# BGI-Qingdao/HAST

Measured on AMD Instinct MI355X. Metric: classified read-bp/sec at k=21, 150bp reads, 200M unique-mers/hap, higher is better.
Workload: dtype u64; 1 GPU; C3 human-trio scale: 200M+200M synthetic 21-mers, 10M barcodes, 150bp reads; k=21, read_len=150, keys_per_hap=200000000, barcodes=10000000, batch_reads=48000000, reads_total=5760000000, minimizer=16, keys=random, collective=none (D2H of counters in timed region), resident_batches=12

## Files before the change

### hast_amd/binding.py

```python
import ctypes as C
import os
import subprocess

import numpy as np

_HERE = os.path.dirname(os.path.abspath(__file__))
_LIB = None

u8p, u32p, u64p, vp = C.POINTER(C.c_uint8), C.POINTER(C.c_uint32), C.POINTER(C.c_uint64), C.c_void_p

STATUS = {0: "OK", 1: "INVALID", 2: "NO_DEVICE", 3: "HIP", 4: "OOM", 5: "TABLE_FULL", 6: "FORMAT", 7: "RCCL", 8: "IO", 9: "UNSUPPORTED"}


class SynthParams(C.Structure):
    _fields_ = [("seed_k", C.c_uint64), ("seed_r", C.c_uint64), ("seed_b", C.c_uint64),
                ("n_keys_per_hap", C.c_uint64), ("n_barcodes", C.c_uint32), ("read_len", C.c_uint32),
                ("k", C.c_uint32), ("reserved", C.c_uint32)]


class KcSynth(C.Structure):
    _fields_ = [("seed", C.c_uint64), ("genome_len", C.c_uint64), ("read_len", C.c_uint32), ("snp_per_1024", C.c_uint32),
                ("err_per_4096", C.c_uint32), ("n_per_4096", C.c_uint32)]


# ... 72 lines not shown
    "hast_dev_free": (C.c_int, [vp, vp]),
    "hast_memcpy_h2d": (C.c_int, [vp, vp, vp, C.c_size_t]),
    "hast_memcpy_d2h": (C.c_int, [vp, vp, vp, C.c_size_t]),
    "hast_memset_d": (C.c_int, [vp, vp, C.c_int, C.c_size_t, vp]),
    "hast_table_reserve": (C.c_int, [vp, C.c_uint64, C.c_double]),
    "hast_table_insert_text": (C.c_int, [vp, C.c_int, C.c_char_p, C.c_size_t, u64p]),
    "hast_table_insert_text_file": (C.c_int, [vp, C.c_int, C.c_char_p, u64p]),
    "hast_ctx_set_text_check": (C.c_int, [vp, C.c_int]),
    "hast_table_insert_keys": (C.c_int, [vp, C.c_int, vp, C.c_size_t]),
    "hast_table_insert_keys_device": (C.c_int, [vp, C.c_int, vp, C.c_size_t, vp]),
    "hast_table_erase": (C.c_int, [vp, vp, C.c_size_t, vp]),
    "hast_table_sizes": (C.c_int, [vp, u64p, u64p]),
    "hast_table_lookup": (C.c_int, [vp, vp, C.c_size_t, vp]),
    "hast_table_save": (C.c_int, [vp, C.c_char_p]),
    "hast_table_load": (C.c_int, [vp, C.c_char_p, C.c_double]),
    "hast_table_file_info": (C.c_int, [C.c_char_p, C.POINTER(C.c_int), u64p]),
    "hast_table_info": (C.c_int, [vp, u64p, u64p]),
    "hast_table_clone": (C.c_int, [vp, vp]),
    "hast_ctx_set_filter": (C.c_int, [vp, C.c_int, C.c_int, C.c_int, C.c_int]),
    "hast_filter_build": (C.c_int, [vp]),
    "hast_filter_info": (C.c_int, [vp, C.POINTER(C.c_int), C.POINTER(C.c_int), C.POINTER(C.c_int), C.POINTER(C.c_int), u64p]),
    "hast_filter_dense": (C.c_int, [vp, C.POINTER(C.c_int)]),
    "hast_filter_request_ceiling": (C.c_int, [vp, C.POINTER(C.c_double)]),
    "hast_counts_resize": (C.c_int, [vp, C.c_size_t]),
    "hast_counts_bind": (C.c_int, [vp, vp, C.c_size_t]),
    "hast_counts_zero": (C.c_int, [vp, vp]),
    "hast_counts_read": (C.c_int, [vp, vp, vp, vp, C.c_size_t]),
    "hast_counts_pack": (C.c_int, [vp, vp, C.c_size_t, vp]),
    "hast_counts_unpack": (C.c_int, [vp, vp, C.c_size_t, vp]),
    "hast_counts_add_votes": (C.c_int, [vp, vp, vp, C.c_size_t, C.c_uint32, vp]),
    "hast_counts_allreduce": (C.c_int, [C.POINTER(vp), C.c_int]),
    "hast_classify_timing": (C.c_int, [vp, C.c_int]),
    "hast_classify_times": (C.c_int, [vp, C.POINTER(C.c_float), C.POINTER(C.c_float), C.c_int, C.POINTER(C.c_int)]),
    "hast_classify_device": (C.c_int, [vp, vp, C.c_size_t, vp, C.c_uint32, vp, vp, C.c_size_t, vp]),
    "hast_classify_batch": (C.c_int, [vp, vp, vp, vp, C.c_size_t, C.c_uint32]),
    "hast_classify_perread_device": (C.c_int, [vp, vp, C.c_size_t, vp, C.c_size_t, vp, vp]),
    "hast_classify_perread": (C.c_int, [vp, vp, vp, C.c_size_t, vp]),
    "hast_batch_begin": (C.c_int, [vp, C.c_size_t, C.c_size_t, C.POINTER(vp), C.POINTER(vp), C.POINTER(vp)]),
    "hast_batch_submit": (C.c_int, [vp, C.c_size_t, C.c_uint32]),
    "hast_names_create": (C.c_int, [vp, C.c_size_t, C.POINTER(vp)]),
    "hast_names_destroy": (None, [vp]),
    "hast_fq_create": (C.c_int, [vp, C.c_size_t, C.c_int, vp, C.POINTER(vp)]),
    "hast_fq_create_ex": (C.c_int, [vp, C.c_size_t, C.c_int, vp, C.c_int, C.POINTER(vp)]),
    "hast_fq_create_striped": (C.c_int, [C.POINTER(vp), C.c_int, C.c_size_t, C.c_int, C.POINTER(vp), C.POINTER(vp)]),
    "hast_fq_create_striped_ex": (C.c_int, [C.POINTER(vp), C.c_int, C.c_size_t, C.c_int, C.POINTER(vp), C.c_int, C.POINTER(vp)]),
    "hast_fq_lanes": (C.c_int, [vp]),
# ... 245 lines not shown
    def filter_build(self):
        _ck(self._lib.hast_filter_build(self._h))

    def filter_request_ceiling(self):
        r = C.c_double()
        _ck(self._lib.hast_filter_request_ceiling(self._h, C.byref(r)))
        return r.value

    def filter_info(self):
        en, m, t, kp, b = C.c_int(), C.c_int(), C.c_int(), C.c_int(), C.c_uint64()
        _ck(self._lib.hast_filter_info(self._h, C.byref(en), C.byref(m), C.byref(t), C.byref(kp), C.byref(b)))
        return bool(en.value), m.value, t.value, kp.value, b.value

    def filter_mode(self):
        en = C.c_int()
        _ck(self._lib.hast_filter_info(self._h, C.byref(en), None, None, None, None))
        return en.value

    def filter_dense(self):
        d = C.c_int()
        _ck(self._lib.hast_filter_dense(self._h, C.byref(d)))
        return bool(d.value)

    def close(self):
        if self._h:
            self._lib.hast_ctx_destroy(self._h)
            self._h = C.c_void_p()

    def __enter__(self):
        return self

    def __exit__(self, *a):
        self.close()

    def __del__(self):
        try:
            self.close()
        except Exception:
            pass

    @property
    def stream(self):
        return self._lib.hast_ctx_stream(self._h)

    def sync(self, stream=None):
        _ck(self._lib.hast_stream_sync(self._h, stream))
# ... 551 lines not shown
```

### hast_amd/csrc/classify_main.cpp

```cpp
#include <getopt.h>
#include <sys/stat.h>
#include <unistd.h>

#include <algorithm>
#include <atomic>
#include <cerrno>
#include <chrono>
#include <deque>
#include <cstdarg>
#include <cstdio>
#include <cstdlib>
#include <cstring>
#include <ctime>
#include <condition_variable>
#include <memory>
#include <mutex>
#include <string>
#include <thread>
#include <string_view>
#include <unordered_map>
#include <vector>

#include "../../include/hast.h"
#include "fq_feed.h"
// ... 1773 lines not shown
    if (o.stats && rs.naming.device_dict)
        stat_line("__stats_dictionary__ on=device dictionaries=%zu ids_limit=%zu ids_from_device=%zu ids_from_host=%zu merge_by_text_s=%.3f texts_merged_to_host=%zu rows_summed_by_text=%zu\n", rs.naming.groups.size(), rs.naming.host_base, rs.n_dev_names, rs.n_host_names, rs.naming.merge_s,
                  rs.naming.merged_to_host, rs.n_rows_summed);
    if (o.stats) {
        const char *nc = getenv("HAST_NAME_CACHE"), *rb = getenv("HAST_GZ_RING_BYTES"), *pg = getenv("HAST_PARK_GB");
        stat_line("__stats_sizes__ name_cache=%s gz_ring_bytes=%s park_gb=%s\n", nc ? nc : "default", rb ? rb : "default", pg ? pg : "default");
    }
    if (o.stats) stat_line("__stats_setup__ waited_for_stream_setup_s=%.3f (inside scrub_sizes_clone_s: .gz inputs opened, FASTQ streams created while the table was built)\n", rs.t_pre_waited);
    for (size_t i = 0; i < rs.ctxs.size(); i++) {
        char sw[512] = "";
        (void)hast_ctx_options(rs.ctxs[i], sw, sizeof(sw));
        if (strstr(sw, "filter_fallback"))
            fprintf(stderr, " WARN : GPU %d (context %zu) had no room for the k-mer filter and probed the table directly (%s)\n", o.devices[i], i, sw);
    }
    if (o.stats) {
        char sw[512] = "";
        (void)hast_ctx_options(rs.ctx, sw, sizeof(sw));
        stat_line("__stats_switches__ %s\n", sw[0] ? sw : "none");
        int f_on = 0, f_m = 0, f_t = 0, f_kp = 0;
        uint64_t f_bytes = 0;
        (void)hast_filter_info(rs.ctx, &f_on, &f_m, &f_t, &f_kp, &f_bytes);
        stat_line("__stats_filter__ mode=%s m=%d t=%d kp=%d bytes=%llu\n", f_on == 2 ? "exact_entries" : f_on == 1 ? "prints" : "off_table_only", f_m, f_t, f_kp,
                  (unsigned long long)f_bytes);
    }
    if (rs.hbm_thread.joinable()) {
        rs.hbm_stop = true;
        rs.hbm_thread.join();
        size_t parked = 0;
        (void)hast_dev_mem_info(rs.ctx, nullptr, nullptr, &parked);
        const size_t fm = rs.hbm_free_min.load(), tot = rs.hbm_total.load();
        if (tot) stat_line("__stats_hbm__ total_bytes=%zu free_min_bytes=%zu in_use_peak_bytes=%zu parked_bytes_at_end=%zu\n", tot, fm, tot - std::min(fm, tot), parked);
    }
    fprintf(stderr, "__END__\n");
    rs.t_printed = now_s();
}

int leave(Run &rs) {
    const Options &o = rs.o;
    const char *preload = getenv("LD_PRELOAD");
    const bool profiled = getenv("ROCP_TOOL_LIBRARIES") || (preload && strstr(preload, "rocprofiler"));
    if (!getenv("HAST_TEARDOWN") && !profiled) {
        if (o.stats) stat_phases(rs, nullptr);
        if (!o.stats_json.empty() && !write_stats_json(o.stats_json)) fprintf(stderr, "classify: cannot write %s\n", o.stats_json.c_str());
        if (fflush(stdout) != 0) die_output();
        fflush(stderr);
        _exit(0);
// ... 51 lines not shown
```

### hast_amd/csrc/hast_api.cpp

```cpp
#include <dlfcn.h>
#include <fcntl.h>
#include <sys/stat.h>
#include <unistd.h>
#include <hip/hip_runtime.h>

#include <algorithm>
#include <chrono>
#include <atomic>
#include <cstdarg>
#include <cstdio>
#include <cstdlib>
#include <cstring>
#include <functional>
#include <map>
#include <mutex>
#include <new>
#include <string>
#include <vector>

#include "../../include/hast.h"
#include "hast_common.h"
#include "hast_device.h"
#include "kc_device.h"
#include "fq_device.h"
// ... 13 lines not shown
    size_t cap_bases = 0, cap_reads = 0;
    hipEvent_t done = nullptr;
    bool in_flight = false;
};

}

struct hast_ctx {
    int device = 0;
    int k = 0;
    int m = 0;
    int n_cu = 256;
    hipStream_t stream = nullptr;
    uint64_t *d_slots = nullptr;
    uint32_t nbuckets = 0;
    unsigned long long *d_counts = nullptr;
    uint32_t *h_errword = nullptr;
    unsigned long long *d_pack = nullptr;
    size_t pack_words = 0;
    size_t n_barcodes = 0;
    bool counts_owned = false;
    uint32_t *d_err = nullptr;
    unsigned long long *d_cnt = nullptr;
    void *d_scratch = nullptr;
    size_t scratch_bytes = 0;
    Staging stage[2];
    unsigned batch_no = 0;
    void *d_seg = nullptr;
    size_t seg_bytes = 0;
    std::vector<hipEvent_t> t_ev;
    size_t t_slots = 0, t_next = 0, t_count = 0;
    uint32_t *d_votes_scratch = nullptr;
    size_t votes_bytes = 0;
    CommitScratch part;
    char *sf_h[2] = {nullptr, nullptr}, *sf_d[2] = {nullptr, nullptr};
    hipEvent_t sf_done[2] = {nullptr, nullptr};
    void *d_filter = nullptr;
    size_t filter_bytes = 0;
    FilterGeom fg{};
    bool filter_valid = false;
    bool use_filter = true;
    size_t filter_fallback_bytes = 0;
    bool test_filter_oom = false;
    int filter_m = 0, filter_t = 0, filter_kp = 0;
    int filter_exact = -1;
    int text_acgt_only = 0;
// ... 197 lines not shown
    if (device < 0 || device >= n) return set_error(HAST_ERR_NO_DEVICE, "device %d not in [0,%d)", device, n);
    HAST_HIP_TRY(hipSetDevice(device));
    tr("hipSetDevice");
    hast_ctx *c = new (std::nothrow) hast_ctx();
    if (!c) return set_error(HAST_ERR_OOM, "host allocation failed");
    c->device = device;
    c->k = k;
    c->m = default_minimizer(k);
    if (const char *e = getenv("HAST_CLASSIFY")) c->use_filter = strcmp(e, "exact") != 0;
    if (const char *e = getenv("HAST_TEST_FILTER_OOM")) c->test_filter_oom = atoi(e) != 0;
    if (const char *e = getenv("HAST_FILTER_M")) c->filter_m = atoi(e);
    if (const char *e = getenv("HAST_FILTER_T")) c->filter_t = atoi(e);
    if (const char *e = getenv("HAST_FILTER_KP")) c->filter_kp = atoi(e);
    if (const char *e = getenv("HAST_FILTER_EXACT")) {
        if (!strcmp(e, "once")) c->exact_env_once = true;
        else c->exact_env_off = atoi(e) == 0;
    }
    if (c->exact_env_off) c->filter_exact = 0;
    else if (c->exact_env_once) c->filter_exact = 1;
    if (const char *e = getenv("HAST_COMMIT")) c->commit_mode = !strcmp(e, "atomic") ? 1 : !strcmp(e, "partition") ? 2 : 0;
    if (const char *e = getenv("HAST_PART_SPAN")) c->part_span = (uint32_t)atoi(e);
    if (const char *e = getenv("HAST_F_GEO")) c->kernel_geo = e[0] != '0';
    if (const char *e = getenv("HAST_F_RL")) c->kernel_rl = e[0] != '0';
    if (const char *e = getenv("HAST_TILE_LDS")) {
        const long v = atol(e);
        if (v >= 4096 && v <= 160 * 1024) c->tile_lds = (size_t)v;
    }
    hipDeviceProp_t prop;
    if (hipGetDeviceProperties(&prop, device) == hipSuccess) c->n_cu = prop.multiProcessorCount;
    tr("hipGetDeviceProperties");
    hast_status st = HAST_OK;
    auto bail = [&](hipError_t he, const char *what) {
        if (he != hipSuccess && st == HAST_OK) st = set_error(HAST_ERR_HIP, "%s: %s", what, hipGetErrorString(he));
    };
    bail(hipStreamCreateWithFlags(&c->stream, hipStreamNonBlocking), "hipStreamCreate");
    tr("hipStreamCreate");
    bail(dev_malloc(&c->d_err, 4 * sizeof(uint32_t)), "dev_malloc(err)");
    tr("first hipMalloc");
    bail(dev_malloc(&c->d_cnt, 8 * sizeof(unsigned long long)), "dev_malloc(cnt)");
    bail(pinned_malloc(reinterpret_cast<void **>(&c->h_errword), 64, hipHostMallocDefault), "pinned_malloc(err word)");
    if (st == HAST_OK) bail(hipMemsetAsync(c->d_err, 0, 4 * sizeof(uint32_t), c->stream), "hipMemset");
    if (st == HAST_OK) bail(hipStreamSynchronize(c->stream), "hipStreamSynchronize");
    tr("first fill + synchronize");
    for (auto &s : c->stage)
        if (st == HAST_OK) bail(hipEventCreateWithFlags(&s.done, hipEventDisableTiming), "hipEventCreate");
    tr("events");
    if (st != HAST_OK) {
        hast_ctx_destroy(c);
        return st;
    }
    *out = c;
    return HAST_OK;
}

void hast_release_parked(void) { release_parked(); }

void hast_ctx_destroy(hast_ctx *c) {
    if (!c) return;
    (void)hipSetDevice(c->device);
    if (c->stream) (void)hipStreamSynchronize(c->stream);
    release_parked();
    for (auto &s : c->stage) {
        if (s.h_bases) (void)hipHostFree(s.h_bases);
        if (s.h_off) (void)hipHostFree(s.h_off);
// ... 787 lines not shown
    uint32_t tr = tr_max;
    if (a.max_pos > 0) {
        double best = -1;
        for (uint32_t t = tr_max; t >= 1 && t + 8 > tr_max; --t) {
            const uint64_t q = (uint64_t)t * a.max_pos, blocks = (q + 63) / 64, slots = filt ? (blocks + 3) / 4 * 4 : (blocks + 7) / 8 * 8;
            const double eff = (double)q / (double)(slots * 64);
            if (eff > best + 1e-9) { best = eff; tr = t; }
        }
    }
    a.tile_reads = tr;
    const size_t smem = per_read * tr + pad;
    if (smem + (filt ? (size_t)kTmerLevelTableWords * 4 : 0) > (160u << 10)) return set_error(HAST_ERR_INVALID, "read_len %u needs %zu B of LDS", read_len, smem);
    auto magic = [](uint64_t qmax, uint32_t d) -> uint32_t {
        if (d <= 1 || qmax * d >= (1ull << 32)) return 0;
        return (uint32_t)((1ull << 32) / d) + 1;
    };
    a.div_magic = magic((uint64_t)tr * a.max_pos + 1024, a.max_pos);
    a.div_mh = magic((uint64_t)tr * a.mh_stride + 1024, a.mh_stride);
    a.div_hw = magic((uint64_t)tr * a.w64 * 2 + 1024, a.w64 * 2);
    a.div_l1g = magic((uint64_t)tr * (a.l1_stride / 4) + 1024, a.l1_stride / 4);
    const uint64_t n_tiles = (n_reads + tr - 1) / tr;
    const int grid = (int)std::min<uint64_t>(n_tiles, (uint64_t)c->n_cu * 8);
    a.tile_queue = c->d_cnt + 3;
    HAST_HIP_TRY(hipMemsetAsync(a.tile_queue, 0, sizeof(unsigned long long), hs));
    hipEvent_t *ev = c->t_slots ? &c->t_ev[3 * (c->t_next % c->t_slots)] : nullptr;
    if (ev) HAST_HIP_TRY(hipEventRecord(ev[0], hs));
    HAST_HIP_TRY(filt ? launch_classify_f(a, grid, smem, (c->kernel_geo ? 1 : 0) | (c->kernel_rl ? 2 : 0), hs) : launch_classify(a, grid, smem, hs));
    if (ev) HAST_HIP_TRY(hipEventRecord(ev[1], hs));
    if (d_barcode_ids) {
        if (hast_status st = commit_run(c, votes_buf, votes16, d_barcode_ids, n_reads, pl, partitioned, hs)) return st;
    }
    if (ev) {
        HAST_HIP_TRY(hipEventRecord(ev[2], hs));
        c->t_next++;
        c->t_count = std::min(c->t_count + 1, c->t_slots);
    }
    return HAST_OK;
}

static hast_status classify_segmented(hast_ctx *c, const uint8_t *d_bases, size_t bases_bytes, const uint64_t *d_offsets, const uint32_t *d_lens,
                                      uint32_t fixed_len, size_t n_reads, int strict, const uint32_t *d_barcode_ids, uint32_t *d_votes_out,
                                      hipStream_t hs);

hast_status hast_ctx_set_filter(hast_ctx *c, int enable, int m, int t, int kp) {
    if (!c) return set_error(HAST_ERR_INVALID, "null context");
    if (m < 0 || m > c->k || m > kFilterMaxM) return set_error(HAST_ERR_INVALID, "filter m=%d out of [0,%d]", m, std::min(c->k, kFilterMaxM));
// ... 23 lines not shown
        if (value && (value < 4096 || value > 160 * 1024)) return set_error(HAST_ERR_INVALID, "tile_lds %ld out of [4096, 163840]", value);
        c->tile_lds = (size_t)value;
    } else if (!strcmp(name, "filter_exact_once")) {
        if (c->filter_exact != 0) c->filter_exact = value ? 1 : (c->exact_env_once ? 1 : -1);
        c->filter_valid = false;
    } else return set_error(HAST_ERR_INVALID, "unknown option %s", name);
    return HAST_OK;
}
hast_status hast_ctx_options(const hast_ctx *c, char *out, size_t cap) {
    if (!c || !out || !cap) return set_error(HAST_ERR_INVALID, "null argument");
    std::string s;
    auto add = [&](const char *n, long v) { s += (s.empty() ? "" : " "); s += n; s += "=" + std::to_string(v); };
    if (!c->use_filter) add("filter", 0);
    if (c->filter_fallback_bytes) add("filter_fallback_table_only_no_room_for_bytes", (long)c->filter_fallback_bytes);
    if (c->filter_exact == 0) add("filter_exact", 0);
    if (c->filter_exact == 1) add("filter_exact_once", 1);
    if (c->filter_m) add("filter_m", c->filter_m);
    if (c->filter_t) add("filter_t", c->filter_t);
    if (c->filter_kp) add("filter_kp", c->filter_kp);
    if (c->commit_mode) add("commit", c->commit_mode);
    if (c->part_span) add("part_span", (long)c->part_span);
    if (!c->kernel_geo) add("kernel_geo", 0);
    if (!c->kernel_rl) add("kernel_rl", 0);
    if (c->tile_lds) add("tile_lds", (long)c->tile_lds);
    if (c->m != default_minimizer_plain(c->k)) add("minimizer", c->m);
    snprintf(out, cap, "%s", s.c_str());
    return HAST_OK;
}

hast_status hast_filter_build(hast_ctx *c) {
    if (hast_status st = need_table(c, 0)) return st;
    if (!c->use_filter) return HAST_OK;
    if (hast_status st = ensure_filter(c, c->stream)) return st;
    HAST_HIP_TRY(hipStreamSynchronize(c->stream));
    return HAST_OK;
}

hast_status hast_filter_info(const hast_ctx *c, int *enabled, int *m, int *t, int *kp, uint64_t *bytes) {
    if (!c) return set_error(HAST_ERR_INVALID, "null context");
    if (enabled) *enabled = !c->use_filter ? 0 : (c->filter_valid && c->fg.exact) ? 2 : 1;
    if (m) *m = c->filter_valid ? c->fg.m : 0;
    if (t) *t = c->filter_valid ? c->fg.t : 0;
    if (kp) *kp = c->filter_valid ? c->fg.kp : 0;
    if (bytes) *bytes = c->filter_valid ? c->filter_bytes : 0;
    return HAST_OK;
}

hast_status hast_filter_dense(const hast_ctx *c, int *dense) {
    if (!c || !dense) return set_error(HAST_ERR_INVALID, "null argument");
    *dense = (c->use_filter && c->filter_valid && c->fg.dense) ? 1 : 0;
    return HAST_OK;
}

hast_status hast_filter_request_ceiling(hast_ctx *c, double *requests_per_s) {
    if (hast_status st = need_table(c, 0)) return st;
    if (!requests_per_s) return set_error(HAST_ERR_INVALID, "null argument");
    if (!c->use_filter) return set_error(HAST_ERR_INVALID, "the filter is off");
    if (hast_status st = ensure_filter(c, c->stream)) return st;
    if (!c->use_filter || !c->d_filter) return set_error(HAST_ERR_INVALID, "no filter (HBM too small for it)");
    const uint64_t nblocks = filter_nblocks(c->fg);
    const int grid = c->n_cu * 8;
    const uint32_t iters = 256;
    uint32_t *d_sink = reinterpret_cast<uint32_t *>(c->d_cnt + 2);
    hipEvent_t e0 = nullptr, e1 = nullptr;
    hipError_t e = hipEventCreate(&e0);
    if (e == hipSuccess) e = hipEventCreate(&e1);
    float best = 0;
    for (int rep = 0; rep < 3 && e == hipSuccess; ++rep) {
        e = hipEventRecord(e0, c->stream);
        if (e == hipSuccess) e = launch_request_ceiling(c->d_filter, nblocks, iters, grid, d_sink, c->stream);
        if (e == hipSuccess) e = hipEventRecord(e1, c->stream);
        if (e == hipSuccess) e = hipEventSynchronize(e1);
        float ms = 0;
// ... 346 lines not shown
```

### hast_amd/csrc/hast_common.h

```cpp
#pragma once
#include <stdint.h>

#include "tmer_level_table.h"

#if defined(__HIPCC__)
#include <hip/hip_runtime.h>
#define HAST_HD __host__ __device__ __forceinline__
#else
#define HAST_HD inline
#endif

namespace hast {

HAST_HD uint32_t base_code(uint32_t c) { return (c & 6u) >> 1; }
HAST_HD uint64_t kmer_mask(int k) { return k >= 32 ? ~0ull : (1ull << (2 * k)) - 1; }

HAST_HD uint64_t kmer_revcomp(uint64_t x, int k) {
    x ^= 0xAAAAAAAAAAAAAAAAull;
#if defined(__HIP_DEVICE_COMPILE__)
    x = __brevll(x);
    x = ((x & 0x5555555555555555ull) << 1) | ((x >> 1) & 0x5555555555555555ull);
#else
    x = ((x & 0x3333333333333333ull) << 2) | ((x >> 2) & 0x3333333333333333ull);
    x = ((x & 0x0F0F0F0F0F0F0F0Full) << 4) | ((x >> 4) & 0x0F0F0F0F0F0F0F0Full);
// ... 136 lines not shown
HAST_HD uint32_t filter_print_of(uint32_t keyhash) {
    const uint32_t f = (keyhash >> 8) & 0xFFFFu;
    return f ? f : 1u;
}
HAST_HD int filter_pos_bits(const FilterGeom &g) {
    int b = 0;
    while ((1u << b) < filter_w(g)) ++b;
    return b;
}
HAST_HD bool filter_exact_fits(const FilterGeom &g) { return g.k <= 32 && g.m <= 14 && 2 * (g.k - g.m) + filter_pos_bits(g) <= 17; }
HAST_HD uint32_t filter_exact_code(uint64_t fwd, uint32_t pm, const FilterGeom &g) {
    const int rb = 2 * (g.k - g.m);
    const uint32_t rest = ((uint32_t)fwd << (2 * pm)) | (uint32_t)(fwd >> (2 * ((uint32_t)g.k - pm)));
    const uint32_t code = (rest & ((1u << rb) - 1u)) | (pm << rb);
    return mul24_forced(code, 0x1D2C5u) & 0x1FFFFu;
}
HAST_HD uint32_t filter_exact_sub(uint32_t code17) { return code17 >> 14; }
HAST_HD uint32_t filter_exact_entry(uint32_t code17, uint32_t tags) { return ((code17 & 0x3FFFu) << 2) | tags; }
constexpr uint32_t kFilterOverflowMark = 0xFFFCu;
constexpr double kFilterDenseMaxLoad = 3.2;
HAST_HD uint32_t filter_dense_pm(uint32_t p, uint32_t w) { return (w - 1u - p) & (w - 1u); }
HAST_HD double filter_dense_load(const FilterGeom &g, uint64_t n_keys) {
    return 2.0 * (double)filter_w(g) * (double)n_keys / ((double)kFilterSubs * (double)filter_nblocks(g));
}
HAST_HD FilterGeom filter_geom_for(int k, uint64_t n_keys, int m_override, int t_override, int kp_override = 0, int exact_mode = -1) {
    FilterGeom g;
    g.k = k;
    int m = k < 8 ? k : 8;
    while (m < k && m < kFilterMaxM && (1ull << (2 * m)) * 3 < 2 * n_keys) ++m;
    if (exact_mode && n_keys >= (16ull << 20) && k - 7 > m && k - 7 <= 14) m = k - 7;
    while (m < kFilterMaxM && k >= m + 9 && 2.0 * (double)n_keys > 2.2 * (double)(1ull << (2 * m))) ++m;
    if (m_override >= 1 && m_override <= k && m_override <= kFilterMaxM) m = m_override;
    g.m = m;
    int kp = k < m + 8 ? k : m + 8;
    if (kp_override >= m && kp_override <= k && kp_override - m < 32) kp = kp_override;
    g.kp = kp;
    const int w = kp - m + 1, r = m < 4 ? m : 4;
    int t = r + (m - r) % w;
    if (t_override >= 1 && t_override <= m) t = t_override;
    g.t = t;
    const int nt = kp - t + 1;
    g.g = nt < 4 ? nt : 4;
    g.wdiv = (65536u / (uint32_t)w) + 1u;
    g.exact = (exact_mode && filter_exact_fits(g)) ? 1 : 0;
    g.choices = (2.0 * (double)n_keys <= 2.2 * (double)(1ull << (2 * m))) ? 1 : 2;
    g.dense = (g.exact && exact_mode < 0 && w <= 8 && (w & (w - 1)) == 0 && filter_dense_load(g, n_keys) <= kFilterDenseMaxLoad) ? 1 : 0;
// ... 80 lines not shown
```

### hast_amd/csrc/hast_device.h

```cpp
#pragma once
#include <hip/hip_runtime.h>
#include <stddef.h>
#include <stdint.h>
#include "commit_plan.h"
#include "hast_common.h"

namespace hast {

struct TableGeom {
    uint32_t nbuckets;
    int k;
    int m;
    int wide;
};

struct ClassifyArgs {
    const uint8_t *bases;
    uint64_t bases_bytes;
    const uint64_t *offsets;
    const uint32_t *lens;
    const uint32_t *seg_read;
    uint32_t *votes;
    uint16_t *votes16;
    unsigned long long *tile_queue;
    const uint64_t *slots;
    uint64_t n_reads;
    const unsigned long long *n_rows_ptr;
    uint32_t nbuckets;
    uint32_t read_len;
    uint32_t max_pos;
    uint32_t w64;
    uint32_t tile_reads;
    uint32_t div_magic;
    uint32_t mh_stride;
    uint32_t div_mh;
    uint32_t div_hw;
    int k;
    int m;
    int wide;
    int strict;
    const void *filter;
    FilterGeom fg;
    uint32_t l1_stride;
    uint32_t div_l1g;
};

hipError_t launch_insert_keys(uint64_t *slots, TableGeom g, const uint64_t *d_keys, size_t n, uint32_t hap,
// ... 35 lines not shown
```

### hast_amd/csrc/hast_filter.hip

```cpp
#include "hast_common.h"
#include "hast_device.h"
#include "hast_devutil.h"

namespace hast {

__device__ __forceinline__ uint32_t sub_load(const uint32_t *w) {
    uint32_t n = 0;
    for (int i = 0; i < kFilterPrints / 2; ++i) {
        const uint32_t v = __hip_atomic_load(&w[i], __ATOMIC_RELAXED, __HIP_MEMORY_SCOPE_AGENT);
        n += (v & 0xFFFFu) != 0;
        n += (v >> 16) != 0;
    }
    return n;
}
__device__ __forceinline__ bool sub_insert(uint32_t *w, uint32_t fp) {
    for (int i = 0; i < kFilterPrints / 2;) {
        const uint32_t v = __hip_atomic_load(&w[i], __ATOMIC_RELAXED, __HIP_MEMORY_SCOPE_AGENT);
        const uint32_t lo = v & 0xFFFFu, hi = v >> 16;
        if (lo == fp || hi == fp) return true;
        uint32_t nv;
        if (lo == 0) nv = v | fp;
        else if (hi == 0) nv = v | (fp << 16);
        else { ++i; continue; }
        if (atomicCAS(&w[i], v, nv) == v) return true;
    }
    return false;
}
__device__ __forceinline__ void sub_mark_overflow(uint32_t *w) {
    uint32_t v = __hip_atomic_load(&w[kFilterPrints / 2 - 1], __ATOMIC_RELAXED, __HIP_MEMORY_SCOPE_AGENT);
    while ((v >> 16) != kFilterOverflowMark) {
        const uint32_t old = atomicCAS(&w[kFilterPrints / 2 - 1], v, (v & 0xFFFFu) | (kFilterOverflowMark << 16));
        if (old == v) break;
        v = old;
    }
}
__device__ __forceinline__ void filter_insert(uint32_t *filt, const FilterGeom g, uint64_t key, uint32_t tags) {
    for (int o = 0; o < 2; ++o) {
        const uint64_t s = o ? kmer_revcomp(key, g.k) : key;
        if (o && s == key) break;
        if (g.exact) {
            const uint32_t pm0 = g.dense ? 0u : filter_sample_pos(s, g), pm1 = g.dense ? filter_w(g) : pm0 + 1u;
            for (uint32_t pm = pm0; pm < pm1; ++pm) {
                const uint32_t blk = filter_block_of((uint32_t)(s >> (2 * (g.k - g.m - (int)pm))) & (uint32_t)kmer_mask(g.m), g.m);
                const uint32_t c17 = filter_exact_code(s, pm, g);
                uint32_t *w = filt + (size_t)blk * (kFilterSubs * kFilterPrints / 2) + filter_exact_sub(c17) * (kFilterPrints / 2);
                if (!sub_insert(w, filter_exact_entry(c17, tags))) sub_mark_overflow(w);
            }
            continue;
        }
        const uint32_t blk = filter_block_of_string(s, g);
        const uint32_t h = filter_keyhash(s), fp = filter_print_of(h);
        uint32_t *b = filt + (size_t)blk * (kFilterSubs * kFilterPrints / 2);
        uint32_t *w1 = b + filter_sub_of(h) * (kFilterPrints / 2), *w2 = b + filter_sub2_of(h) * (kFilterPrints / 2);
        if (g.choices == 1) {
            (void)sub_insert(w1, fp);
            continue;
        }
        bool there = false;
        for (int i = 0; i < kFilterPrints / 2 && !there; ++i) {
            const uint32_t v = __hip_atomic_load(&w2[i], __ATOMIC_RELAXED, __HIP_MEMORY_SCOPE_AGENT);
            there = (v & 0xFFFFu) == fp || (v >> 16) == fp;
        }
        if (there) continue;
        if (w1 != w2 && sub_load(w2) < sub_load(w1)) { uint32_t *t = w1; w1 = w2; w2 = t; }
        if (!sub_insert(w1, fp) && w1 != w2) (void)sub_insert(w2, fp);
    }
}

__global__ void __launch_bounds__(256) k_filter_build(const uint64_t *slots, size_t nslots, uint32_t *filt, FilterGeom g, int wide) {
// ... 68 lines not shown
    uint32_t *s_len = reinterpret_cast<uint32_t *>(s_off + TR);
    uint32_t *s_flag = s_len + TR;
    uint32_t *s_q = s_flag + TR;
    const uint32_t IW = 2 * W64 + 1;
    uint32_t *s_inv = s_q + 4 * 3 * kQCap;

    const uint32_t tid = threadIdx.x;
    const uint32_t lane = tid & 63;
    const uint32_t wave = (uint32_t)__builtin_amdgcn_readfirstlane((int)(tid >> 6));
    uint32_t *q_lo = s_q + wave * 3 * kQCap, *q_hi = q_lo + kQCap, *q_rd = q_hi + kQCap;
    typedef GeoConst<GEO> GC;
    FilterGeom fg = a.fg;
    if (GEO) {
        fg.k = GC::k; fg.m = GC::m; fg.t = GC::t; fg.kp = GC::kp;
        fg.g = 4;
        fg.wdiv = 65536u / (uint32_t)(GC::kp - GC::m + 1) + 1u;
    }
    const int K = GEO ? GC::k : a.k, M = fg.m, T = fg.t;
    const uint32_t G = (uint32_t)fg.g, W = filter_w(fg), NT = filter_nt(fg);
    const uint32_t ntc = NTC ? (uint32_t)NTC : (NT + G - 1) / G;
    const uint32_t kshift = 64 - 2 * K, tshift = 64 - 2 * T;
    const uint32_t mmask = (uint32_t)kmer_mask(M);
    const uint32_t nb = a.nbuckets;
    const uint64_t n_rows = a.n_rows_ptr ? min((uint64_t)*a.n_rows_ptr, (uint64_t)a.n_reads) : a.n_reads;
    const uint64_t n_tiles = (n_rows + TR - 1) / TR;
    const uintptr_t base_addr = reinterpret_cast<uintptr_t>(a.bases);
    const uintptr_t end_addr = (base_addr + a.bases_bytes + 3) & ~(uintptr_t)3;
    const u32x4f *filt = reinterpret_cast<const u32x4f *>(a.filter);
    const u64x2f *tab0 = reinterpret_cast<const u64x2f *>(a.slots);

    if (!DENSE)
        for (uint32_t i = tid; i < kTmerLevelTableWords; i += kThreadsF) s_lvl[i] = kTmerLevelWords[i];
    if (tid == 0) *s_tile = atomicAdd(a.tile_queue, 1ull);
    __syncthreads();
    for (;;) {
        const uint64_t tile = *s_tile;
        if (tile >= n_tiles) break;
        const uint64_t r0 = tile * TR;
        const uint32_t tra = (uint32_t)((n_rows - r0 < TR) ? (n_rows - r0) : TR);

        if (STRICT && tid == 0) *s_dirty = 0;
        if (tid < tra) {
            uint64_t off, len;
            const uint32_t rlen = RLC ? (uint32_t)RL : a.read_len;
            if (a.offsets) { off = a.offsets[r0 + tid]; len = a.lens ? a.lens[r0 + tid] : a.offsets[r0 + tid + 1] - off; }
            else           { off = (r0 + tid) * (uint64_t)rlen; len = rlen; }
// ... 93 lines not shown
                const uint32_t tm = (uint32_t)window_bits(s_pack + (size_t)r * WS, q, tshift);
                const uint32_t e = valid ? tmer_order_lds(s_lvl, tm, q) : 0xFFFFFFFFu;
                uint32_t mn = e;
                if (G >= 2) mn = min(mn, (uint32_t)__shfl_down((int)e, 1));
                if (G >= 3) mn = min(mn, (uint32_t)__shfl_down((int)e, 2));
                if (lane < step && in) s_l1[idx] = mn;
            }
        }
        if (!DENSE) __syncthreads();
        if (!STRICT) {
            if (tid < tra && s_flag[tid]) s_len[tid] = 0;
            __syncthreads();
        }

        const uint32_t P = RLC ? (uint32_t)(RL - GC0::k + 1) : a.max_pos;
        const bool tile_dirty = STRICT && __builtin_amdgcn_readfirstlane((int)*s_dirty) != 0;
        uint32_t qn = 0;
        auto drain = [&](uint32_t cnt) {
            const bool act = lane < cnt;
            const uint32_t e = act ? qn - cnt + lane : 0;
            const unsigned long long key = kmer_canon(((unsigned long long)q_hi[e] << 32) | q_lo[e], K);
            const uint32_t rd = q_rd[e];
            qn -= cnt;
            for (int pass = 0; pass < (WIDE ? 2 : 1); ++pass) {
                const u64x2f *tab = tab0 + (WIDE ? (size_t)pass * nb * kPieces : 0);
                const unsigned long long want = WIDE ? key : (key << 2);
                uint32_t b = act ? home_bucket(key, K, a.m, nb) : 0;
                bool pending = act;
                uint32_t step = 0;
                while (__any(pending)) {
                    u64x2f s[kPieces];
#pragma unroll
                    for (int l = 0; l < kPieces; ++l) s[l] = u64x2f{kEmptySlot, kEmptySlot};
                    if (pending) {
#pragma unroll
                        for (int l = 0; l < kPieces; ++l) s[l] = tab[(size_t)b * kPieces + l];
                    }
                    unsigned long long hit_slot = 0;
                    bool hit = false;
#pragma unroll
                    for (int l = 0; l < kPieces; ++l) {
                        if ((WIDE ? s[l].x : (s[l].x & ~3ull)) == want) { hit_slot = s[l].x; hit = true; }
                        if ((WIDE ? s[l].y : (s[l].y & ~3ull)) == want) { hit_slot = s[l].y; hit = true; }
                    }
                    hit = hit && pending;
                    if (hit) {
// ... 31 lines not shown
                    ok = ok & clean;
                    okm &= ballot64(clean);
                }
            }
            const unsigned long long fwd = window_bits(s_pack + mul24(r, WS), p, kshift);
            uint32_t pm;
            if (DENSE) {
                pm = filter_dense_pm(p, W);
            } else {
                const uint32_t *l1 = s_l1 + mul24(r, L1S) + p;
                uint32_t x = l1[0];
                if (NTC) {
#pragma unroll
                    for (int c = 1; c + 1 < (NTC ? NTC : 1); ++c) x = min(x, l1[c * 4]);
                } else {
                    for (uint32_t c = 1; c + 1 < ntc; ++c) x = min(x, l1[c * G]);
                }
                if (ntc > 1) x = min(x, l1[NT - G]);
                const uint32_t xr = ((x & 0xFFFu) - p) & 63u;
                pm = (GEO && (W & (W - 1)) == 0) ? (xr & (W - 1)) : xr - mul24(mul24(xr, fg.wdiv) >> 16, W);
            }
            const uint32_t mm = (uint32_t)(fwd >> (2 * ((uint32_t)(K - M) - pm))) & mmask;
            uint32_t fb = ok ? filter_block_of(mm, M) : 0xFFFFFFFFu;
            const uint32_t h = EXACT ? filter_exact_code(fwd, pm, fg) : filter_keyhash(fwd);
            const uint32_t anchor = okm ? (uint32_t)__builtin_amdgcn_readlane((int)fb, (int)__builtin_ctzll(okm)) : last_fb;
            last_fb = anchor;
            fb = ok ? fb : anchor;
            if (EXACT) {
                B.v = filt[(fb << 3) | filter_exact_sub(h)];
                B.fpw = mul24((h & 0x3FFFu) ^ 0x3FFFu, 0x00040004u);
            } else {
                B.v = filt[(size_t)fb * kFilterSubs + filter_sub_of(h)];
                if (TWO) B.v2 = filt[(size_t)fb * kFilterSubs + filter_sub2_of(h)];
                const uint32_t fp = filter_print_of(h);
                B.fpw = fp | (fp << 16);
            }
            B.klo = (uint32_t)fwd;
            B.khi = (uint32_t)(fwd >> 32);
            B.meta = r | (ok ? 0x80000000u : 0u);
            pos = pos + 64 < q_end ? pos + 64 : q_end;
            if (P >= 64) {
                cp += 64;
                const bool wrap = cp >= P;
                cp -= wrap ? P : 0u;
                cr += wrap ? 1u : 0u;
            } else locate();
        };
        auto finish = [&](Blk &B) {
            bool pos;
            if (EXACT) {
                const uint32_t mx = pk_max_u16(pk_max_u16(B.v.x ^ B.fpw, B.v.y ^ B.fpw), pk_max_u16(B.v.z ^ B.fpw, B.v.w ^ B.fpw));
                const uint32_t m16 = max(mx >> 16, mx & 0xFFFFu);
                const bool valid = (int)B.meta < 0;
                const bool hit = valid && m16 >= 0xFFFDu;
                if (hit) atomicAdd(&s_vote[B.meta & 0xFFFFu], (unsigned long long)(m16 & 1u) | ((unsigned long long)((m16 >> 1) & 1u) << 32));
                pos = valid && !hit && (B.v.w >> 16) == kFilterOverflowMark;
            } else {
            uint32_t acc = pk_min_u16(pk_min_u16(B.v.x ^ B.fpw, B.v.y ^ B.fpw), pk_min_u16(B.v.z ^ B.fpw, B.v.w ^ B.fpw));
            bool full = (B.v.w >> 16) != 0;
            if (TWO) {
                acc = pk_min_u16(acc, pk_min_u16(pk_min_u16(B.v2.x ^ B.fpw, B.v2.y ^ B.fpw), pk_min_u16(B.v2.z ^ B.fpw, B.v2.w ^ B.fpw)));
                full = full && (B.v2.w >> 16) != 0;
            }
            const bool match = ((acc - 0x00010001u) & ~acc & 0x80008000u) != 0;
            pos = (int)B.meta < 0 && (match || full);
            }
            const unsigned long long pmask = ballot64(pos);
            if (pmask) {
                const uint32_t at = qn + lanes_below(pmask);
                if (pos) {
                    q_lo[at] = B.klo;
                    q_hi[at] = B.khi;
                    q_rd[at] = B.meta & 0xFFFFu;
                }
                qn += (uint32_t)__popcll(pmask);
                if (qn >= 64) drain(64);
            }
        };
        {
            const uint32_t rpw = (tra + 3) >> 2;
            const uint32_t r_first = wave * rpw < tra ? wave * rpw : tra, r_last = r_first + rpw < tra ? r_first + rpw : tra;
            pos = r_first * P;
            q_end = r_last * P;
            locate();
            if (pos < q_end) {
                Blk A, B;
                start(A);
                while (pos < q_end) {
                    start(B);
                    finish(A);
// ... 119 lines not shown
```

### include/hast.h

```cpp
#ifndef HAST_H
#define HAST_H
#include <stddef.h>
#include <stdint.h>

#ifdef __cplusplus
extern "C" {
#endif

typedef enum {
    HAST_OK = 0,
    HAST_ERR_INVALID = 1,
    HAST_ERR_NO_DEVICE = 2,
    HAST_ERR_HIP = 3,
    HAST_ERR_OOM = 4,
    HAST_ERR_TABLE_FULL = 5,
    HAST_ERR_FORMAT = 6,
    HAST_ERR_RCCL = 7,
    HAST_ERR_IO = 8,
    HAST_ERR_UNSUPPORTED = 9
} hast_status;

typedef struct hast_ctx hast_ctx;
typedef void *hast_stream;

// ... 29 lines not shown
hast_status hast_table_insert_keys(hast_ctx *, int hap, const uint64_t *canon_keys, size_t n);
hast_status hast_table_insert_keys_device(hast_ctx *, int hap, const uint64_t *d_canon_keys, size_t n,
                                          hast_stream);

hast_status hast_table_erase(hast_ctx *, const uint64_t *canon_keys, size_t n, uint8_t *out_hit);

hast_status hast_table_sizes(hast_ctx *, uint64_t *n_hap0, uint64_t *n_hap1);

hast_status hast_table_lookup(hast_ctx *, const uint64_t *canon_keys, size_t n, uint8_t *out_tags);

hast_status hast_table_save(hast_ctx *, const char *path);
hast_status hast_table_load(hast_ctx *, const char *path, double load_factor);
hast_status hast_table_file_info(const char *path, int *k_out, uint64_t *n_keys_out);

hast_status hast_table_clone(hast_ctx *dst, hast_ctx *src);

hast_status hast_table_info(const hast_ctx *, uint64_t *n_buckets, uint64_t *bytes);

hast_status hast_ctx_set_filter(hast_ctx *, int enable, int m, int t, int kp);
hast_status hast_filter_build(hast_ctx *);
hast_status hast_filter_info(const hast_ctx *, int *enabled, int *m, int *t, int *kp, uint64_t *bytes);
hast_status hast_filter_dense(const hast_ctx *, int *dense);
hast_status hast_filter_request_ceiling(hast_ctx *, double *requests_per_s);

hast_status hast_counts_resize(hast_ctx *, size_t n_barcodes);
hast_status hast_counts_bind(hast_ctx *, uint64_t *d_counts, size_t n_barcodes);
hast_status hast_counts_zero(hast_ctx *, hast_stream);
hast_status hast_counts_read(hast_ctx *, uint64_t *c0, uint64_t *c1, uint64_t *neg, size_t n_barcodes);
hast_status hast_counts_read_range(hast_ctx *, size_t first, size_t n, uint64_t *c0, uint64_t *c1, uint64_t *neg);
hast_status hast_counts_pack(hast_ctx *, uint64_t *d_packed, size_t n_barcodes, hast_stream);
hast_status hast_counts_unpack(hast_ctx *, const uint64_t *d_packed, size_t n_barcodes, hast_stream);
hast_status hast_counts_add_votes(hast_ctx *, const uint32_t *d_votes, const uint32_t *d_barcode_ids, size_t n_reads,
                                  uint32_t max_votes, hast_stream);
hast_status hast_counts_allreduce(hast_ctx *const *ctxs, int n_ctx);
hast_status hast_counts_permute(hast_ctx *, const uint32_t *perm, size_t n_perm, size_t n_new);

hast_status hast_classify_device(hast_ctx *, const uint8_t *d_bases, size_t bases_bytes,
                                 const uint64_t *d_offsets, uint32_t read_len,
                                 const uint32_t *d_barcode_ids, uint32_t *d_votes,
                                 size_t n_reads, hast_stream);
hast_status hast_classify_timing(hast_ctx *, int n_slots);
hast_status hast_classify_times(hast_ctx *, float *classify_ms, float *commit_ms, int max, int *n_out);
hast_status hast_classify_batch(hast_ctx *, const uint8_t *bases, const uint64_t *offsets,
                                const uint32_t *barcode_ids, size_t n_reads, uint32_t max_read_len);

hast_status hast_classify_perread_device(hast_ctx *, const uint8_t *d_bases, size_t bases_bytes,
// ... 257 lines not shown
```

Before: 386.0 billion bp/s.

## Add dense filter encoding with overflow signature marks to cut table probes

For the dense exact-filter layout, entries are now encoded with a new position-aware code. Sub-blocks that overflow keep a two-bit Bloom-style signature in their last slot instead of a blanket overflow mark. During classification, windows that land on an overflowed sub-block are sent to the hash table only if their signature bits are present, which cuts table look-ups caused by overflow. An opt-in counter of windows sent to the table is also added, with an API and stats line to read it. The change adds a serial readlane loop per wave for positive lanes, and it depends on the filter build and the query using the same encoding.

```diff
diff --git a/hast_amd/binding.py b/hast_amd/binding.py
--- a/hast_amd/binding.py
+++ b/hast_amd/binding.py
@@ -118,6 +118,7 @@
     "hast_filter_info": (C.c_int, [vp, C.POINTER(C.c_int), C.POINTER(C.c_int), C.POINTER(C.c_int), C.POINTER(C.c_int), u64p]),
     "hast_filter_dense": (C.c_int, [vp, C.POINTER(C.c_int)]),
     "hast_filter_request_ceiling": (C.c_int, [vp, C.POINTER(C.c_double)]),
+    "hast_filter_lookups": (C.c_int, [vp, C.POINTER(C.c_uint64)]),
     "hast_counts_resize": (C.c_int, [vp, C.c_size_t]),
     "hast_counts_bind": (C.c_int, [vp, vp, C.c_size_t]),
     "hast_counts_zero": (C.c_int, [vp, vp]),
@@ -409,6 +410,11 @@
         _ck(self._lib.hast_filter_dense(self._h, C.byref(d)))
         return bool(d.value)
 
+    def filter_lookups(self):
+        n = C.c_uint64()
+        _ck(self._lib.hast_filter_lookups(self._h, C.byref(n)))
+        return n.value
+
     def close(self):
         if self._h:
             self._lib.hast_ctx_destroy(self._h)
diff --git a/hast_amd/csrc/classify_main.cpp b/hast_amd/csrc/classify_main.cpp
--- a/hast_amd/csrc/classify_main.cpp
+++ b/hast_amd/csrc/classify_main.cpp
@@ -1819,6 +1819,11 @@
         (void)hast_filter_info(rs.ctx, &f_on, &f_m, &f_t, &f_kp, &f_bytes);
         stat_line("__stats_filter__ mode=%s m=%d t=%d kp=%d bytes=%llu\n", f_on == 2 ? "exact_entries" : f_on == 1 ? "prints" : "off_table_only", f_m, f_t, f_kp,
                   (unsigned long long)f_bytes);
+        uint64_t lk = 0, lk_all = 0;
+        bool counted = false;
+        for (hast_ctx *cx : rs.ctxs)
+            if (hast_filter_lookups(cx, &lk) == HAST_OK) { lk_all += lk; counted = true; }
+        if (counted) stat_line("__stats_lookups__ windows_sent_to_table=%llu\n", (unsigned long long)lk_all);
     }
     if (rs.hbm_thread.joinable()) {
         rs.hbm_stop = true;
diff --git a/hast_amd/csrc/hast_api.cpp b/hast_amd/csrc/hast_api.cpp
--- a/hast_amd/csrc/hast_api.cpp
+++ b/hast_amd/csrc/hast_api.cpp
@@ -59,6 +59,7 @@
     bool counts_owned = false;
     uint32_t *d_err = nullptr;
     unsigned long long *d_cnt = nullptr;
+    bool count_lookups = false;
     void *d_scratch = nullptr;
     size_t scratch_bytes = 0;
     Staging stage[2];
@@ -302,6 +303,7 @@
     if (const char *e = getenv("HAST_PART_SPAN")) c->part_span = (uint32_t)atoi(e);
     if (const char *e = getenv("HAST_F_GEO")) c->kernel_geo = e[0] != '0';
     if (const char *e = getenv("HAST_F_RL")) c->kernel_rl = e[0] != '0';
+    if (const char *e = getenv("HAST_COUNT_LOOKUPS")) c->count_lookups = atoi(e) != 0;
     if (const char *e = getenv("HAST_TILE_LDS")) {
         const long v = atol(e);
         if (v >= 4096 && v <= 160 * 1024) c->tile_lds = (size_t)v;
@@ -320,6 +322,7 @@
     bail(dev_malloc(&c->d_cnt, 8 * sizeof(unsigned long long)), "dev_malloc(cnt)");
     bail(pinned_malloc(reinterpret_cast<void **>(&c->h_errword), 64, hipHostMallocDefault), "pinned_malloc(err word)");
     if (st == HAST_OK) bail(hipMemsetAsync(c->d_err, 0, 4 * sizeof(uint32_t), c->stream), "hipMemset");
+    if (st == HAST_OK) bail(hipMemsetAsync(c->d_cnt, 0, 8 * sizeof(unsigned long long), c->stream), "hipMemset");
     if (st == HAST_OK) bail(hipStreamSynchronize(c->stream), "hipStreamSynchronize");
     tr("first fill + synchronize");
     for (auto &s : c->stage)
@@ -1153,6 +1156,7 @@
     const uint64_t n_tiles = (n_reads + tr - 1) / tr;
     const int grid = (int)std::min<uint64_t>(n_tiles, (uint64_t)c->n_cu * 8);
     a.tile_queue = c->d_cnt + 3;
+    a.lookups = (filt && c->count_lookups) ? c->d_cnt + 5 : nullptr;
     HAST_HIP_TRY(hipMemsetAsync(a.tile_queue, 0, sizeof(unsigned long long), hs));
     hipEvent_t *ev = c->t_slots ? &c->t_ev[3 * (c->t_next % c->t_slots)] : nullptr;
     if (ev) HAST_HIP_TRY(hipEventRecord(ev[0], hs));
@@ -1222,6 +1226,7 @@
     if (c->part_span) add("part_span", (long)c->part_span);
     if (!c->kernel_geo) add("kernel_geo", 0);
     if (!c->kernel_rl) add("kernel_rl", 0);
+    if (c->count_lookups) add("count_lookups", 1);
     if (c->tile_lds) add("tile_lds", (long)c->tile_lds);
     if (c->m != default_minimizer_plain(c->k)) add("minimizer", c->m);
     snprintf(out, cap, "%s", s.c_str());
@@ -1249,6 +1254,17 @@
 hast_status hast_filter_dense(const hast_ctx *c, int *dense) {
     if (!c || !dense) return set_error(HAST_ERR_INVALID, "null argument");
     *dense = (c->use_filter && c->filter_valid && c->fg.dense) ? 1 : 0;
+    return HAST_OK;
+}
+
+hast_status hast_filter_lookups(hast_ctx *c, uint64_t *n) {
+    if (hast_status st = use(c)) return st;
+    if (!n) return set_error(HAST_ERR_INVALID, "null argument");
+    if (!c->count_lookups) return set_error(HAST_ERR_INVALID, "look-ups are not counted (HAST_COUNT_LOOKUPS=1 when the context is created)");
+    unsigned long long v = 0;
+    HAST_HIP_TRY(hipDeviceSynchronize());
+    HAST_HIP_TRY(hipMemcpy(&v, c->d_cnt + 5, sizeof(v), hipMemcpyDeviceToHost));
+    *n = v;
     return HAST_OK;
 }
 
diff --git a/hast_amd/csrc/hast_common.h b/hast_amd/csrc/hast_common.h
--- a/hast_amd/csrc/hast_common.h
+++ b/hast_amd/csrc/hast_common.h
@@ -182,6 +182,60 @@
 HAST_HD uint32_t filter_dense_pm(uint32_t p, uint32_t w) { return (w - 1u - p) & (w - 1u); }
 HAST_HD double filter_dense_load(const FilterGeom &g, uint64_t n_keys) {
     return 2.0 * (double)filter_w(g) * (double)n_keys / ((double)kFilterSubs * (double)filter_nblocks(g));
+}
+HAST_HD uint32_t filter_dense_code(uint64_t fwd, uint32_t pm, const FilterGeom &g, uint32_t pos_bits) {
+    const int rb = 2 * (g.k - g.m);
+    const uint32_t rot = ((uint32_t)fwd << (2 * pm)) | (uint32_t)(fwd >> (2 * ((uint32_t)g.k - pm)));
+    const uint32_t rest = rot & ((1u << rb) - 1u);
+    return (((pm | (rest << pos_bits)) & 7u) << 14) | (rest >> (3u - pos_bits));
+}
+HAST_HD uint32_t filter_dense_pm_of(uint32_t sub, uint32_t pos_bits) { return sub & ((1u << pos_bits) - 1u); }
+HAST_HD uint32_t filter_dense_rest_of(uint32_t sub, uint32_t stored, uint32_t pos_bits) { return (stored << (3u - pos_bits)) | (sub >> pos_bits); }
+HAST_HD uint32_t filter_mark_sig(uint32_t stored14) {
+    const uint32_t h = (stored14 & 0x3FFFu) * 0x9E3779B1u;
+    const uint32_t a = ((h >> 24) * 14u) >> 8;
+    const uint32_t b = (((h >> 16) & 0xFFu) * 13u) >> 8;
+    const uint32_t b2 = a + 1u + b;
+    return (1u << a) | (1u << (b2 >= 14u ? b2 - 14u : b2));
+}
+HAST_HD bool filter_is_mark(uint32_t slot7) { return slot7 != 0 && (slot7 & 3u) == 0; }
+HAST_HD uint32_t filter_word_load(uint32_t *p) {
+#if defined(__HIP_DEVICE_COMPILE__)
+    return __hip_atomic_load(p, __ATOMIC_RELAXED, __HIP_MEMORY_SCOPE_AGENT);
+#else
+    return *p;
+#endif
+}
+HAST_HD uint32_t filter_word_cas(uint32_t *p, uint32_t expect, uint32_t v) {
+#if defined(__HIP_DEVICE_COMPILE__)
+    return atomicCAS(p, expect, v);
+#else
+    const uint32_t old = *p;
+    if (old == expect) *p = v;
+    return old;
+#endif
+}
+HAST_HD void filter_dense_file(uint32_t *w, uint32_t entry) {
+    for (int i = 0; i < kFilterPrints / 2;) {
+        const uint32_t v = filter_word_load(&w[i]);
+        const uint32_t lo = v & 0xFFFFu, hi = v >> 16;
+        if (lo == entry || hi == entry) return;
+        uint32_t nv;
+        if (lo == 0) nv = v | entry;
+        else if (hi == 0) nv = v | (entry << 16);
+        else { ++i; continue; }
+        if (filter_word_cas(&w[i], v, nv) == v) return;
+    }
+    const uint32_t sig = filter_mark_sig(entry >> 2) << 2;
+    uint32_t v = filter_word_load(&w[kFilterPrints / 2 - 1]);
+    for (;;) {
+        const uint32_t hi = v >> 16;
+        const uint32_t nh = (hi & 3u) ? (sig | (filter_mark_sig(hi >> 2) << 2)) : (hi | sig);
+        if (nh == hi) return;
+        const uint32_t old = filter_word_cas(&w[kFilterPrints / 2 - 1], v, (v & 0xFFFFu) | (nh << 16));
+        if (old == v) return;
+        v = old;
+    }
 }
 HAST_HD FilterGeom filter_geom_for(int k, uint64_t n_keys, int m_override, int t_override, int kp_override = 0, int exact_mode = -1) {
     FilterGeom g;
diff --git a/hast_amd/csrc/hast_device.h b/hast_amd/csrc/hast_device.h
--- a/hast_amd/csrc/hast_device.h
+++ b/hast_amd/csrc/hast_device.h
@@ -23,6 +23,7 @@
     uint32_t *votes;
     uint16_t *votes16;
     unsigned long long *tile_queue;
+    unsigned long long *lookups;
     const uint64_t *slots;
     uint64_t n_reads;
     const unsigned long long *n_rows_ptr;
diff --git a/hast_amd/csrc/hast_filter.hip b/hast_amd/csrc/hast_filter.hip
--- a/hast_amd/csrc/hast_filter.hip
+++ b/hast_amd/csrc/hast_filter.hip
@@ -40,11 +40,13 @@
         if (o && s == key) break;
         if (g.exact) {
             const uint32_t pm0 = g.dense ? 0u : filter_sample_pos(s, g), pm1 = g.dense ? filter_w(g) : pm0 + 1u;
+            const uint32_t pb = (uint32_t)filter_pos_bits(g);
             for (uint32_t pm = pm0; pm < pm1; ++pm) {
                 const uint32_t blk = filter_block_of((uint32_t)(s >> (2 * (g.k - g.m - (int)pm))) & (uint32_t)kmer_mask(g.m), g.m);
-                const uint32_t c17 = filter_exact_code(s, pm, g);
+                const uint32_t c17 = g.dense ? filter_dense_code(s, pm, g, pb) : filter_exact_code(s, pm, g);
                 uint32_t *w = filt + (size_t)blk * (kFilterSubs * kFilterPrints / 2) + filter_exact_sub(c17) * (kFilterPrints / 2);
-                if (!sub_insert(w, filter_exact_entry(c17, tags))) sub_mark_overflow(w);
+                if (g.dense) filter_dense_file(w, filter_exact_entry(c17, tags));
+                else if (!sub_insert(w, filter_exact_entry(c17, tags))) sub_mark_overflow(w);
             }
             continue;
         }
@@ -159,6 +161,7 @@
     const uint32_t kshift = 64 - 2 * K, tshift = 64 - 2 * T;
     const uint32_t mmask = (uint32_t)kmer_mask(M);
     const uint32_t nb = a.nbuckets;
+    const uint32_t PB = DENSE ? (uint32_t)filter_pos_bits(fg) : 0u;
     const uint64_t n_rows = a.n_rows_ptr ? min((uint64_t)*a.n_rows_ptr, (uint64_t)a.n_reads) : a.n_reads;
     const uint64_t n_tiles = (n_rows + TR - 1) / TR;
     const uintptr_t base_addr = reinterpret_cast<uintptr_t>(a.bases);
@@ -298,6 +301,7 @@
             const unsigned long long key = kmer_canon(((unsigned long long)q_hi[e] << 32) | q_lo[e], K);
             const uint32_t rd = q_rd[e];
             qn -= cnt;
+            if (EXACT && a.lookups && lane == 0) atomicAdd(a.lookups, (unsigned long long)cnt);
             for (int pass = 0; pass < (WIDE ? 2 : 1); ++pass) {
                 const u64x2f *tab = tab0 + (WIDE ? (size_t)pass * nb * kPieces : 0);
                 const unsigned long long want = WIDE ? key : (key << 2);
@@ -375,7 +379,7 @@
             }
             const uint32_t mm = (uint32_t)(fwd >> (2 * ((uint32_t)(K - M) - pm))) & mmask;
             uint32_t fb = ok ? filter_block_of(mm, M) : 0xFFFFFFFFu;
-            const uint32_t h = EXACT ? filter_exact_code(fwd, pm, fg) : filter_keyhash(fwd);
+            const uint32_t h = DENSE ? filter_dense_code(fwd, pm, fg, PB) : EXACT ? filter_exact_code(fwd, pm, fg) : filter_keyhash(fwd);
             const uint32_t anchor = okm ? (uint32_t)__builtin_amdgcn_readlane((int)fb, (int)__builtin_ctzll(okm)) : last_fb;
             last_fb = anchor;
             fb = ok ? fb : anchor;
@@ -407,7 +411,7 @@
                 const bool valid = (int)B.meta < 0;
                 const bool hit = valid && m16 >= 0xFFFDu;
                 if (hit) atomicAdd(&s_vote[B.meta & 0xFFFFu], (unsigned long long)(m16 & 1u) | ((unsigned long long)((m16 >> 1) & 1u) << 32));
-                pos = valid && !hit && (B.v.w >> 16) == kFilterOverflowMark;
+                pos = valid && !hit && (DENSE ? (B.v.w & 0x30000u) == 0 && B.v.w >= 0x10000u : (B.v.w >> 16) == kFilterOverflowMark);
             } else {
             uint32_t acc = pk_min_u16(pk_min_u16(B.v.x ^ B.fpw, B.v.y ^ B.fpw), pk_min_u16(B.v.z ^ B.fpw, B.v.w ^ B.fpw));
             bool full = (B.v.w >> 16) != 0;
@@ -418,7 +422,18 @@
             const bool match = ((acc - 0x00010001u) & ~acc & 0x80008000u) != 0;
             pos = (int)B.meta < 0 && (match || full);
             }
-            const unsigned long long pmask = ballot64(pos);
+            unsigned long long pmask = ballot64(pos);
+            if (DENSE && pmask) {
+                unsigned long long keep = 0;
+                for (unsigned long long rest = pmask; rest; rest &= rest - 1) {
+                    const int l = (int)__builtin_ctzll(rest);
+                    const uint32_t f = (uint32_t)__builtin_amdgcn_readlane((int)B.fpw, l), s7 = (uint32_t)__builtin_amdgcn_readlane((int)B.v.w, l) >> 16;
+                    const uint32_t sig = filter_mark_sig(~(f >> 2) & 0x3FFFu) << 2;
+                    if ((s7 & sig) == sig) keep |= 1ull << l;
+                }
+                pmask = keep;
+                pos = __builtin_amdgcn_inverse_ballot_w64(keep);
+            }
             if (pmask) {
                 const uint32_t at = qn + lanes_below(pmask);
                 if (pos) {
diff --git a/include/hast.h b/include/hast.h
--- a/include/hast.h
+++ b/include/hast.h
@@ -75,6 +75,7 @@
 hast_status hast_filter_info(const hast_ctx *, int *enabled, int *m, int *t, int *kp, uint64_t *bytes);
 hast_status hast_filter_dense(const hast_ctx *, int *dense);
 hast_status hast_filter_request_ceiling(hast_ctx *, double *requests_per_s);
+hast_status hast_filter_lookups(hast_ctx *, uint64_t *n);
 
 hast_status hast_counts_resize(hast_ctx *, size_t n_barcodes);
 hast_status hast_counts_bind(hast_ctx *, uint64_t *d_counts, size_t n_barcodes);
```

After: 393.7 billion bp/s, median of 6. 1.02x the previous value.
